# huangjh-pub/di-fusion

Hardware: AMD Instinct MI355X
Metric: frames/s integrate+decode+mesh, 640x480 synthetic stream (higher is better)
Workload: dtype f32

## Files before the change

### di_fusion_amd/_lib.py

```python
from __future__ import annotations

import ctypes
import os
from ctypes import POINTER, Structure, c_float, c_int32, c_int64, c_uint8, c_void_p
from pathlib import Path

PKG = Path(__file__).resolve().parent
LIB_PATH = Path(os.environ["DIF_LIB"]) if os.environ.get("DIF_LIB") else PKG / "libdifusion.so"

C_N_OCCUPIED, C_OVERFLOW, C_ALLOC_NEW, C_M, C_C, C_ITEMS, C_K, C_B, C_VH, C_T, C_QUERY_M, C_N_KEPT, C_CACHE_T, C_CACHE_KEPT, C_EXPORT_N, C_WORK, C_CACHE_DEAD, C_CACHE_LIVE, C_OPT_ROWS, C_OPT_VOXELS, C_HALO_L, C_HALO_R, C_HALO_TICKET, C_DEFERRED = range(24)
C_STAMP = 31
SYNC_FUSED, SYNC_FRONT_DONE, SYNC_WORDS = 0, 32, 64
FC_COUNT = 32
C_COUNT = 32
PROF_NAMES = ["encode", "decode_lattice", "decode_points", "mc_count", "mc_emit", "halo_export", "halo_merge"]
PROF_COUNT = 8
LATENT_DIM = 29

ERRORS = {-1: "DIF_EINVAL (bad argument)", -2: "DIF_ELAUNCH (HIP launch/runtime failure)", -3: "DIF_ENOSPACE (workspace too small)"}


class DifMap(Structure):
    _fields_ = [("nx", c_int32), ("ny", c_int32), ("nz", c_int32),
                ("bound_min", c_float * 3), ("voxel_size", c_float),
                ("prune_min_vox_obs", c_int32), ("ignore_count_th", c_float), ("encoder_count_th", c_float),
                ("capacity", c_int64),
                ("indexer", c_void_p), ("latent_vecs", c_void_p), ("latent_vecs_pos", c_void_p),
# ... 100 lines not shown
    "dif_query_decode": (c_int32, [POINTER(DifMap), POINTER(DifWeights), c_void_p, c_int64, c_void_p, c_void_p, c_void_p, c_void_p, c_void_p]),
    "dif_query_grad_scatter": (c_int32, [c_void_p, c_void_p, c_void_p, c_int64, c_void_p, c_void_p]),
    "dif_query_grad_gather": (c_int32, [c_void_p, c_void_p, c_void_p, c_int64, c_void_p, c_void_p]),
    "dif_export_records": (c_int32, [POINTER(DifMap), c_void_p, c_int64, c_int32, c_int32, c_int32, c_void_p, c_void_p]),
    "dif_merge_records": (c_int32, [POINTER(DifMap), c_void_p, c_int64, c_int32, c_void_p, c_void_p]),
    "dif_export_halo": (c_int32, [POINTER(DifMap), c_void_p, c_int64, c_int32, c_int32, c_void_p, c_void_p]),
    "dif_merge_halo": (c_int32, [POINTER(DifMap), c_void_p, c_int64, c_void_p, c_void_p]),
    "dif_export_halo_delta": (c_int32, [POINTER(DifMap), c_void_p, c_void_p, c_int64, c_void_p, c_void_p]),
    "dif_halo_lists_reset": (c_int32, [POINTER(DifMap), c_void_p, c_void_p, c_void_p, c_void_p]),
    "dif_merge_halo2": (c_int32, [POINTER(DifMap), c_void_p, c_int64, c_void_p, c_int64, c_void_p, c_void_p, c_void_p]),
    "dif_profile_enable": (c_int32, [c_int32]),
    "dif_profile_read": (c_int32, [POINTER(ctypes.c_double), POINTER(c_int64), c_int32]),
    "dif_profile_dump": (c_int64, [POINTER(c_int32), POINTER(c_float), c_int64, c_int32]),
    "dif_read_counters": (c_int32, [POINTER(DifMap), POINTER(c_int32), c_void_p]),
    "dif_test_mc_grid_cap": (c_int32, [c_int32]),
    "dif_test_sdma_mode": (c_int32, [c_int32]),
    "dif_sdma_info": (c_int32, [POINTER(c_int32)]),
    "dif_test_handoff": (c_int32, [c_int32, c_int32, c_int32, c_int32, POINTER(c_int64)]),
    "dif_queues_independent": (c_int32, [c_void_p, c_void_p]),
    "dif_mesh_cache_export_sdma": (c_int32, [POINTER(DifExtractBuffers), c_int64, c_int64, c_void_p, c_void_p, c_void_p]),
    "dif_sdf_hg_workspace_bytes": (c_int64, [c_int64]),
    "dif_sdf_hg": (c_int32, [POINTER(DifMap), POINTER(DifWeights), c_void_p, c_int64, POINTER(DifSdfHg), c_void_p, c_int64, c_void_p, c_void_p,
                             c_int64, c_void_p]),
    "dif_gradient_xy": (c_int32, [c_void_p, c_int32, c_int32, c_void_p, c_void_p]),
    "dif_photo_pyramid": (c_int32, [c_void_p, c_void_p, c_int32, c_int32, POINTER(DifPhotoPyramid), c_void_p]),
    "dif_rgb_odometry": (c_int32, [c_void_p, c_void_p, c_void_p, c_void_p, c_void_p, c_int32, c_int32, POINTER(DifRgbHg), c_void_p, c_void_p,
                                   c_void_p]),
    "dif_rgb_hg_workspace_bytes": (c_int64, []),
    "dif_rgb_hg": (c_int32, [c_void_p, c_void_p, c_void_p, c_void_p, c_void_p, c_int32, c_int32, POINTER(DifRgbHg), c_void_p, c_int64, c_void_p,
                             c_void_p, c_int64, c_void_p]),
# ... 67 lines not shown
```

### di_fusion_amd/csrc/difusion.hip

```cpp
#include <cstdlib>
#include <cstdio>
#include <cstring>
#include <mutex>
#include <atomic>
#include <chrono>
#include <vector>
#include <hip/hip_runtime.h>
#include <hsa/hsa.h>
#include <hsa/hsa_ext_amd.h>
#include <dlfcn.h>

#include "common.hip.h"
#include "mlp.hip.h"
#include "mc_tables.inc"

using namespace dif;

namespace {

constexpr int L = DIF_LATENT_DIM;

__device__ __constant__ int c_mc_edge_table[256];
__device__ __constant__ unsigned long long c_mc_tri_packed[256];
bool g_tables_uploaded[64] = {};
// ... 442 lines not shown
    }
    return DIF_OK;
}

static int integrate_impl(const dif_map_t* map, const dif_weights_t* w, const float* xyz, const float* normal, int64_t N, uint8_t* unq_mask,
                          void* wsp, int64_t ws_bytes, const FrameSource* src, void* stream_) {
    if (!map || !w || !w->enc_packed || w->enc_packed_floats != ENC_FLOATS || N < 0 || !map->grid_tot) return DIF_EINVAL;
    if (N == 0) return DIF_OK;
    if (!src && (!xyz || !normal)) return DIF_EINVAL;
    IntegratePlan P;
    const int rc = integrate_plan(map, w, xyz, normal, N, unq_mask, wsp, ws_bytes, src, P);
    if (rc != DIF_OK) return rc;
    hipStream_t s = (hipStream_t)stream_;
    const int nb_pts = (int)((N + DIF_BLOCK - 1) / DIF_BLOCK);
    const int nb_x = P.has_pending ? DIF_EXPORT_WGS : 0;
    if (P.overlap && wait_word(s, map->sync_words + DIF_SYNC_FUSED, map->frame_seq - 1) != DIF_OK) return DIF_ELAUNCH;
    if (src)
        hipLaunchKernelGGL(k_unproject_voxel_count, dim3(nb_pts + nb_x), dim3(DIF_BLOCK), 0, s, P.uvc, ImageGeo{src->H, src->W, src->fx, src->fy, src->cx, src->cy}, nb_x);
    else
        hipLaunchKernelGGL(k_voxel_count, dim3(nb_pts), dim3(DIF_BLOCK), 0, s, P.uvc.g, xyz, N, P.uvc.pt_lin, P.uvc.frame_count, P.uvc.counters, P.uvc.px_lo,
                           P.uvc.px_hi);
    hipLaunchKernelGGL(k_prune_mark, dim3(nb_pts + nb_x), dim3(DIF_BLOCK), 0, s, P.prune, N, nb_x);
    DIF_CHECK_LAUNCH();
    if (launch_counted_scan(P.alloc, (int)((P.grid + 31) / 32), P.alloc_tot, s) != DIF_OK) return DIF_ELAUNCH;
    hipLaunchKernelGGL(k_focus_gather, dim3(nb_pts + nb_x), dim3(DIF_BLOCK), 0, s, P.gather, N, (src && src->W % 16 == 0 && src->H % 16 == 0) ? src->W : 0, nb_x);
    DIF_CHECK_LAUNCH();
    {
        const bool x6 = w->enc_x6_packed && w->enc_x6_packed_bytes == E6_BYTES;
        const size_t lds_bytes = x6 ? (size_t)E6_BYTES : (size_t)ENC_FLOATS * 4;
        if (encoder_attributes() != DIF_OK) return DIF_ELAUNCH;
        const EncArgs& e = P.enc;
        ProfScope prof(DIF_PROF_ENCODE, s);
        const int enc_grid = P.overlap ? overlap_encoder_cus() : num_cus();
        if (x6)
            hipLaunchKernelGGL(k_encode<true>, dim3(enc_grid), dim3(ENC_X6_THREADS), lds_bytes, s, e.g, (const float*)w->enc_x6_packed, e.src.xyz, e.src.normal, e.src.frame,
                               e.src.im, N, e.pair_list, e.rec_dir, e.rec_next, e.rec, e.upd_list, e.counters, e.dirty, e.dirty_tot);
        else
            hipLaunchKernelGGL(k_encode<false>, dim3(enc_grid), dim3(512), lds_bytes, s, e.g, w->enc_packed, e.src.xyz, e.src.normal, e.src.frame,
                               e.src.im, N, e.pair_list, e.rec_dir, e.rec_next, e.rec, e.upd_list, e.counters, e.dirty, e.dirty_tot);
        DIF_CHECK_LAUNCH();
    }
    hipStream_t sf = s;
    if (P.overlap) {
        sf = (hipStream_t)map->fuse_stream;
        hipLaunchKernelGGL(k_publish_word, dim3(1), dim3(64), 0, s, map->sync_words + DIF_SYNC_FRONT_DONE, (uint32_t)map->frame_seq);
        if (wait_word(sf, map->sync_words + DIF_SYNC_FRONT_DONE, map->frame_seq) != DIF_OK) return DIF_ELAUNCH;
    }
    hipLaunchKernelGGL(k_fuse, dim3(grid_for(map->capacity * 32, DIF_BLOCK, 256)), dim3(DIF_BLOCK), 0, sf, P.fuse);
    DIF_CHECK_LAUNCH();
    return DIF_OK;
}

int dif_integrate(const dif_map_t* map, const dif_weights_t* w, const float* xyz, const float* normal, int64_t N, uint8_t* unq_mask,
                  void* wsp, int64_t ws_bytes, void* stream_) {
    return integrate_impl(map, w, xyz, normal, N, unq_mask, wsp, ws_bytes, nullptr, stream_);
}

int dif_integrate_frame(const dif_map_t* map, const dif_weights_t* w, const dif_frame_t* frame_dev, int32_t H, int32_t W, float fx, float fy, float cx,
                        float cy, float* xyz_world, float* normal_world, uint8_t* unq_mask, void* wsp, int64_t ws_bytes, void* stream_) {
    if (!frame_dev || H <= 0 || W <= 0 || (xyz_world == nullptr) != (normal_world == nullptr)) return DIF_EINVAL;
    FrameSource src{frame_dev, H, W, fx, fy, cx, cy};
    return integrate_impl(map, w, xyz_world, normal_world, (int64_t)H * W, unq_mask, wsp, ws_bytes, &src, stream_);
}
// ... 368 lines not shown
}

static void mc_onepass_args(McArgs& a, const dif_map_t* map, const dif_extract_buffers_t* buf, bool defer) {
    a.tri_start = map->tri_start; a.tri_n = map->tri_n; a.tri_count = buf->tri_count; a.tri_offset = nullptr;
    if (!defer && buf->out_tri && buf->out_id && buf->out_std) {
        a.out_tri = buf->out_tri; a.out_id = buf->out_id; a.out_std = buf->out_std; a.out_capacity = buf->out_capacity;
    }
}

static FinishArgs finish_args_of(const dif_map_t* map, const dif_extract_buffers_t* buf, bool fused_scan, bool onepass, bool exported, bool defer) {
    int32_t* const super_sum = buf->chunk_sum ? buf->chunk_sum + (buf->max_voxels + 255) / 256 : nullptr;
    const bool ov = overlapped(map);
    return FinishArgs{buf->occ_slot, map->vbm, map->counters, buf->max_triangles, buf->cache_capacity, buf->cache_tri, buf->cache_id, buf->cache_std,
                      ExtractOut{buf->counters_out, buf->out_tri, buf->out_id, buf->out_std, buf->out_capacity, (exported || defer) ? 1 : 0,
                                 defer ? (dif_pending_export_t*)map->pending_export : nullptr, buf->stamp, defer ? buf->export_notify : nullptr},
                      (fused_scan && !onepass) ? buf->chunk_sum : nullptr, super_sum, map->dirty_tot, (int)((map->capacity + DIF_BLOCK - 1) / DIF_BLOCK),
                      onepass ? buf->mc_status : nullptr, onepass ? buf->mc_status + (buf->max_voxels + 3) / 4 : nullptr,
                      ov ? map->frame_counters : nullptr};
}

static int voxel_decode_attributes() {
    static bool attr_set[64] = {};
    int dev = 0; (void)hipGetDevice(&dev);
    if (dev < 64 && !attr_set[dev]) {
        const int fp32_bytes = (int)(((size_t)((DEC_LDS_FLOATS + 3) & ~3) + 4 * VD_WAVE_LDS_FLOATS) * 4);
        const int x6_bytes = (int)((size_t)X6_LDS_BYTES + 4 * VD_WAVE_LDS_FLOATS * 4);
        if (hipFuncSetAttribute((const void*)k_decode_voxels<false>, hipFuncAttributeMaxDynamicSharedMemorySize, fp32_bytes) != hipSuccess) return DIF_ELAUNCH;
        if (hipFuncSetAttribute((const void*)k_decode_voxels<true>, hipFuncAttributeMaxDynamicSharedMemorySize, x6_bytes) != hipSuccess) return DIF_ELAUNCH;
        if (hipFuncSetAttribute((const void*)k_decode_refine_x6, hipFuncAttributeMaxDynamicSharedMemorySize, (int)X6_LDS_BYTES) != hipSuccess) return DIF_ELAUNCH;
        if (hipFuncSetAttribute((const void*)k_decode_voxels_batch<true>, hipFuncAttributeMaxDynamicSharedMemorySize, x6_bytes) != hipSuccess) return DIF_ELAUNCH;
        if (hipFuncSetAttribute((const void*)k_decode_refine_x6_batch, hipFuncAttributeMaxDynamicSharedMemorySize, (int)X6_LDS_BYTES) != hipSuccess) return DIF_ELAUNCH;
        attr_set[dev] = true;
    }
    return DIF_OK;
}

static std::atomic<int> g_mc_grid_cap{0};
int dif_test_mc_grid_cap(int32_t n) { return g_mc_grid_cap.exchange(n > 0 ? n : 0); }

static int mc_onepass_setup(const McArgs& a, size_t& lds_bytes, int& grid1, int64_t max_voxels) {
    if (upload_tables() != DIF_OK) return DIF_ELAUNCH;
    const int r = a.R / 2, nc = (r + 1) * (r + 1) * (r + 1);
    lds_bytes = (size_t)(DIF_BLOCK / 64) * MC_ONEPASS_WAVE_LDS_FLOATS(nc) * sizeof(float);
    if (lds_bytes > 128 * 1024) return DIF_EINVAL;
    static bool attr_set1[64] = {};
    int dev = 0; (void)hipGetDevice(&dev);
    if (dev < 64 && !attr_set1[dev]) {
        if (hipFuncSetAttribute((const void*)k_marching_cubes_onepass<0>, hipFuncAttributeMaxDynamicSharedMemorySize, 128 * 1024) != hipSuccess) return DIF_ELAUNCH;
        if (hipFuncSetAttribute((const void*)k_marching_cubes_onepass<4>, hipFuncAttributeMaxDynamicSharedMemorySize, 128 * 1024) != hipSuccess) return DIF_ELAUNCH;
        if (hipFuncSetAttribute((const void*)k_marching_cubes_onepass_batch<0>, hipFuncAttributeMaxDynamicSharedMemorySize, 128 * 1024) != hipSuccess) return DIF_ELAUNCH;
        if (hipFuncSetAttribute((const void*)k_marching_cubes_onepass_batch<4>, hipFuncAttributeMaxDynamicSharedMemorySize, 128 * 1024) != hipSuccess) return DIF_ELAUNCH;
        attr_set1[dev] = true;
    }
// ... 15 lines not shown
    const int* n_slots = map->counters + DIF_C_N_OCCUPIED;
    if (!map->grid_tot) return DIF_EINVAL;
    const GridMarks bits = grid_marks_of(map);
    if (buf->cache_capacity <= 0 || buf->cache_capacity >= ((int64_t)1 << 31) || !buf->cache_tri || !buf->cache_id || !buf->cache_std || !buf->cache_alive)
        return DIF_EINVAL;
    if (!map->tri_start || !map->tri_n) return DIF_EINVAL;
    hipStream_t s = (hipStream_t)stream_;
    const int64_t grid = (int64_t)map->nx * map->ny * map->nz;
    Geo g = geo_of(map);
    int* C = map->counters;
    const bool ov = overlapped(map);
    if (ov && (!overlap_ok(map) || no_cache || defer_export_of(map, buf) || s != (hipStream_t)map->fuse_stream)) return DIF_EINVAL;
    const ExtractGeo e = extract_geo(resolution);
    const int r = e.r, R = e.R, l = e.l, R3 = e.R3;
    if (buf->max_voxels * (int64_t)R3 >= ((int64_t)1 << 31)) return DIF_EINVAL;
    const double sample_a = e.sample_a, sample_b = e.sample_b;

    {
        const DirtySet ds = dirty_set_of(map, buf, no_cache);
        const bool tiled = ds.tiled;
        if (tiled) {
            hipLaunchKernelGGL(k_mark_halo_dirty, dim3(grid_for(map->capacity, DIF_BLOCK, 256)), dim3(DIF_BLOCK), 0, s, g, map->ignore_count_th, map->dirty,
                               (const int64_t*)map->latent_vecs_pos, (const int64_t*)map->indexer, (const float*)map->voxel_obs_count, bits,
                               n_slots, ds.own_lin_lo, ds.own_lin_hi);
            DIF_CHECK_LAUNCH();
        }
        {
            DirtyFunctor f{ds};
            if (map->dirty_tot && !no_cache && !tiled && map->capacity > 4096 && map->capacity % DIF_BLOCK == 0) {
                hipLaunchKernelGGL(k_dirty_scan, dim3((int)(map->capacity / DIF_BLOCK)), dim3(DIF_BLOCK), 0, s, ds, n_slots, (const int*)map->dirty_tot,
                                   ov ? map->sync_words + DIF_SYNC_FUSED : nullptr, (int)map->frame_seq);
                DIF_CHECK_LAUNCH();
            } else if (ov) {
                return DIF_EINVAL;
            } else if (map->dirty_tot && !no_cache && !tiled) {
                if (launch_counted_scan_bounded(f, n_slots, map->capacity, map->dirty_tot, s) != DIF_OK) return DIF_ELAUNCH;
            } else if (launch_scan(f, n_slots, 0, map->capacity, buf->block_tmp, s) != DIF_OK) return DIF_ELAUNCH;
        }
    }
    {
        OccFunctor f{map->grid_bits, map->indexer, buf->occ_slot, map->vbm, C, buf->max_voxels};
        if (launch_counted_scan(f, (int)((grid + 31) / 32), map->grid_tot, s) != DIF_OK) return DIF_ELAUNCH;
    }
    int rc;
    if (fast && l * l * l <= VD_MAX_L3 && R * R <= VD_MAX_R2) {
        if (!w->dec_packed || w->dec_packed_floats != DEC_FLOATS) return DIF_EINVAL;
        const bool fold = w->dec_fold_packed && w->dec_fold_packed_floats == DECF_FLOATS && buf->fold_table;
        const VoxelDecodeArgs V = voxel_decode_args_of(map, w, buf, e, fold);
        const bool x6 = fold && w->dec_x6_packed && w->dec_x6_packed_bytes == X6_BYTES;
        const size_t lds_bytes = x6 ? (size_t)X6_LDS_BYTES + 4 * VD_WAVE_LDS_FLOATS * 4
                                    : ((size_t)((DEC_LDS_FLOATS + 3) & ~3) + 4 * VD_WAVE_LDS_FLOATS) * 4;
        if (voxel_decode_attributes() != DIF_OK) return DIF_ELAUNCH;
        int64_t blocks = (buf->max_voxels + 3) / 4;
        if (blocks > num_cus()) blocks = num_cus();
        {
            ProfScope prof(DIF_PROF_DECODE_LATTICE, s);
            if (x6) hipLaunchKernelGGL(k_decode_voxels<true>, dim3((int)blocks), dim3(512), lds_bytes, s, V, (const float*)w->dec_x6_packed);
            else hipLaunchKernelGGL(k_decode_voxels<false>, dim3((int)blocks), dim3(512), lds_bytes, s, V, w->dec_packed);
        }
        DIF_CHECK_LAUNCH();
        const DecodeArgs Rf = refine_args_of(map, buf, e, fold);
        if (x6) {
            int64_t rblocks = (buf->max_voxels * (int64_t)(R3 / 32) + 7) / 8;
// ... 32 lines not shown
    return extract_mesh_part(map, buf, e, max_std, no_cache, scale_vertices, s);
}

static int extract_mesh_part(const dif_map_t* map, const dif_extract_buffers_t* buf, const ExtractGeo& e, float max_std, int32_t no_cache,
                             int32_t scale_vertices, hipStream_t s) {
    int* C = map->counters;
    const int r = e.r;
    int rc;
    McArgs a = mc_args_of(map, buf, e, max_std, scale_vertices);
    if (no_cache) {
        if (hipMemsetAsync(C + DIF_C_CACHE_T, 0, sizeof(int), s) != hipSuccess) return DIF_ELAUNCH;
        if (hipMemsetAsync(C + DIF_C_CACHE_DEAD, 0, sizeof(int), s) != hipSuccess) return DIF_ELAUNCH;
        if (hipMemsetAsync(map->tri_n, 0, sizeof(int32_t) * (size_t)map->capacity, s) != hipSuccess) return DIF_ELAUNCH;
    }
    const bool defer = defer_export_of(map, buf);
    const bool fused_scan = buf->chunk_sum && buf->max_voxels <= ((int64_t)1 << 24);
    int32_t* const super_sum = buf->chunk_sum ? buf->chunk_sum + (buf->max_voxels + 255) / 256 : nullptr;
    const bool onepass = fused_scan && buf->mc_status && r * r * r <= 64;
    if (onepass) {
        mc_onepass_args(a, map, buf, defer);
        size_t lds_bytes; int grid1;
        rc = mc_onepass_setup(a, lds_bytes, grid1, buf->max_voxels);
        if (rc != DIF_OK) return rc;
        {
            ProfScope prof(DIF_PROF_MC_COUNT, s);
            if (r == 4) hipLaunchKernelGGL(k_marching_cubes_onepass<4>, dim3(grid1), dim3(DIF_BLOCK), lds_bytes, s, a, buf->mc_status, buf->mc_status + (buf->max_voxels + 3) / 4);
            else hipLaunchKernelGGL(k_marching_cubes_onepass<0>, dim3(grid1), dim3(DIF_BLOCK), lds_bytes, s, a, buf->mc_status, buf->mc_status + (buf->max_voxels + 3) / 4);
        }
        DIF_CHECK_LAUNCH();
    } else if (fused_scan) {
        a.chunk_sum = buf->chunk_sum; a.super_sum = super_sum; a.tri_start = map->tri_start; a.tri_n = map->tri_n;
        a.tri_count = buf->tri_count; a.tri_offset = nullptr;
        size_t lds_bytes; int blocks;
        rc = mc_setup(a, lds_bytes, blocks, buf->max_voxels);
        if (rc != DIF_OK) return rc;
        {
            ProfScope prof(DIF_PROF_MC_COUNT, s);
            hipLaunchKernelGGL(k_marching_cubes<false>, dim3(blocks), dim3(DIF_BLOCK), lds_bytes, s, a);
        }
        {
            ProfScope prof(DIF_PROF_MC_EMIT, s);
            hipLaunchKernelGGL(k_marching_cubes<true>, dim3(blocks), dim3(DIF_BLOCK), lds_bytes, s, a);
        }
        DIF_CHECK_LAUNCH();
    } else {
        TriScanFunctor ts{};
        ts.valid_blocks = buf->valid_blocks; ts.indexer = map->indexer; ts.tri_start = map->tri_start; ts.tri_n = map->tri_n; ts.alive = buf->cache_alive;
        ts.new_limit = buf->max_triangles; ts.capacity = buf->cache_capacity;
        rc = mc_count_and_scan(a, buf->max_voxels, buf->tri_count, buf->tri_offset, buf->block_tmp, C, ts, s);
        if (rc != DIF_OK) return rc;
        rc = mc_emit(a, buf->max_voxels, buf->tri_count, buf->tri_offset, s);
        if (rc != DIF_OK) return rc;
    }
    hipLaunchKernelGGL(k_extract_finish, dim3(grid_for(buf->max_voxels, DIF_BLOCK, 256)), dim3(DIF_BLOCK), 0, s,
                       finish_args_of(map, buf, fused_scan, onepass, onepass && a.out_tri, defer));
    DIF_CHECK_LAUNCH();
    return DIF_OK;
}

int dif_extract_streams(const dif_stream_frame_t* st, int32_t S, const dif_weights_t* w, int32_t resolution, float max_std, int32_t scale_vertices,
                        void* stream_) {
    if (!batch_maps_ok(st, S) || !w || resolution < 1 || resolution > 4) return DIF_EINVAL;
    const ExtractGeo e = extract_geo(resolution);
    if (e.l * e.l * e.l > VD_MAX_L3 || e.R * e.R > VD_MAX_R2 || e.r * e.r * e.r > 64) return DIF_EINVAL;
    if (!w->dec_packed || w->dec_packed_floats != DEC_FLOATS || !w->dec_fold_packed || w->dec_fold_packed_floats != DECF_FLOATS || !w->dec_x6_packed ||
        w->dec_x6_packed_bytes != X6_BYTES)
        return DIF_EINVAL;
    const dif_map_t* m0 = st[0].map;
// ... 706 lines not shown
```

### di_fusion_amd/csrc/kernels_extract.hip.h

```cpp
#pragma once

__device__ __forceinline__ void mark_confident_nbhd(const Geo& g, int lin, float ignore_th, const int64_t* __restrict__ indexer,
                                                    const float* __restrict__ obs, const GridMarks& marks) {
    const uint32_t* bits = marks.bits;
    int ix, iy, iz;
    unlinearize(g, lin, ix, iy, iz);
    int cand[7];
    cand[0] = lin;
    cand[1] = linearize(g, clampi(ix - 1, 0, g.nx - 1), iy, iz);
    cand[2] = linearize(g, clampi(ix + 1, 0, g.nx - 1), iy, iz);
    cand[3] = linearize(g, ix, clampi(iy - 1, 0, g.ny - 1), iz);
    cand[4] = linearize(g, ix, clampi(iy + 1, 0, g.ny - 1), iz);
    cand[5] = linearize(g, ix, iy, clampi(iz - 1, 0, g.nz - 1));
    cand[6] = linearize(g, ix, iy, clampi(iz + 1, 0, g.nz - 1));
    int64_t slot[7];
#pragma unroll
    for (int c = 0; c < 7; ++c) slot[c] = indexer[cand[c]];
    float w[7];
#pragma unroll
    for (int c = 0; c < 7; ++c) w[c] = slot[c] >= 0 ? obs[slot[c]] : ignore_th;
    uint32_t word[7];
#pragma unroll
    for (int c = 0; c < 7; ++c) word[c] = (w[c] > ignore_th) ? bits[cand[c] >> 5] : 0xFFFFFFFFu;
    uint32_t prev[7];
// ... 47 lines not shown
    __device__ int count(int s) const { return ((a.no_cache || a.dirty[s]) && a.owned(s)) ? 1 : 0; }
    __device__ void emit(int s, int offset) const {
        a.dirty[s] = 0;
        if (offset >= a.max_voxels) return;
        const int lin = (int)a.pos[s];
        a.valid_blocks[offset] = lin;
        mark_confident_nbhd(a.g, lin, a.ignore_th, a.indexer, a.obs, a.bits);
    }
    __device__ void finish(int total) const {
        if (total > a.max_voxels) { total = (int)a.max_voxels; a.counters[DIF_C_OVERFLOW] = 2; }
        a.counters[DIF_C_K] = total;
        a.counters[DIF_C_DEFERRED] = 0;
    }
};

__device__ __forceinline__ void dirty_scan_body(const DirtySet& a, const int* __restrict__ n_ptr, const int* __restrict__ block_tot,
                                                uint32_t* __restrict__ fused_word, int seq) {
    __shared__ int smem[8];
    if (fused_word && blockIdx.x == 0 && threadIdx.x == 0) __hip_atomic_store(fused_word, (uint32_t)seq, __ATOMIC_RELAXED, __HIP_MEMORY_SCOPE_AGENT);
    const int s = (int)blockIdx.x * DIF_BLOCK + (int)threadIdx.x;
    const bool flag = a.dirty[s] != 0;
    if (!__syncthreads_or((int)flag) && blockIdx.x != 0) return;
    int before = 0, all = 0;
    const int n_blk = (int)gridDim.x;
    for (int b = (int)threadIdx.x; b < n_blk; b += DIF_BLOCK) {
        const int t = block_tot[b];
        all += t;
        if (b < (int)blockIdx.x) before += t;
    }
    const GridMarks& marks = a.bits;
    int lin = 0, cand[7];
    uint32_t word[7];
#pragma unroll
    for (int c = 0; c < 7; ++c) { cand[c] = 0; word[c] = 0xFFFFFFFFu; }
// ... 40 lines not shown
                prev[c] = (word[c] & b) ? 0xFFFFFFFFu : atomicOr(marks.bits + (cand[c] >> 5), b);
            }
#pragma unroll
            for (int c = 0; c < 7; ++c)
                if (!(prev[c] & (1u << (cand[c] & 31)))) atomicAdd(marks.tot + (cand[c] >> 5) / marks.per_words, 1);
        }
    }
    if (blockIdx.x == 0 && threadIdx.x == 0) {
        int t = total;
        if (t > a.max_voxels) { t = (int)a.max_voxels; a.counters[DIF_C_OVERFLOW] = 2; }
        a.counters[DIF_C_K] = t;
        a.counters[DIF_C_DEFERRED] = 0;
    }
}

__global__ void __launch_bounds__(DIF_BLOCK) k_dirty_scan(DirtySet a, const int* __restrict__ n_ptr, const int* __restrict__ block_tot, uint32_t* __restrict__ fused_word, int seq) {
    dirty_scan_body(a, n_ptr, block_tot, fused_word, seq);
}
struct DirtyScanArgs { DirtySet a; const int* n_ptr; const int* block_tot; };
__global__ void __launch_bounds__(DIF_BLOCK) k_dirty_scan_batch(Batch<DirtyScanArgs> b) {
    const DirtyScanArgs& a = b.s[blockIdx.y];
    dirty_scan_body(a.a, a.n_ptr, a.block_tot, nullptr, 0);
}
__global__ void k_publish_word(uint32_t* __restrict__ word, uint32_t value) {
    if (threadIdx.x == 0) __hip_atomic_store(word, value, __ATOMIC_RELAXED, __HIP_MEMORY_SCOPE_AGENT);
}

struct OccFunctor {
    uint32_t* bits;
    const int64_t* indexer;
    int32_t* occ_slot;
    int32_t* vbm;
    int* counters;
    int64_t max_voxels;
    __device__ int count(int w) const { return __popc(bits[w]); }
    __device__ void emit(int w, int offset) const {
        uint32_t word = bits[w];
// ... 374 lines not shown
        __syncthreads();
    }
}

struct VoxelDecodeArgs {
    const int32_t* occ_slot;
    const float* latent;
    Lattice low;
    int R;
    float* cube_sdf;
    float* cube_std;
    int32_t* refine_list;
    int* counters;
    const float* fold_w;
    float* fold_table;
};

#define VD_MAX_L3 64
#define VD_MAX_R2 64
#define VD_WAVE_LDS_FLOATS (2 * VD_MAX_L3 + 2 * 256)

#ifdef DIF_TRACE
__device__ unsigned long long g_vd_trace[2048 * 8];
#define VD_STAMP(slot) do { if (lane_id() == 0) g_vd_trace[((threadIdx.x >> 6) * gridDim.x + blockIdx.x) * 8 + (slot)] = wall_clock64(); } while (0)
#else
#define VD_STAMP(slot) do { } while (0)
#endif

template <bool X6, int NS>
__device__ __forceinline__ void decode_voxels_body(const BatchN<VoxelDecodeArgs, NS>& AB, int S, const float* __restrict__ wblob) {
// ... 117 lines not shown
            int32_t* const refine_list = A.refine_list;
            while (sel) {
                const int jz = __ffs((int)sel) - 1;
                sel &= sel - 1;
                refine_list[o++] = (int32_t)(e0 + jz);
            }
        }
        __syncthreads();
        VD_STAMP(4);
    }
    VD_STAMP(5);
}

template <bool X6>
__global__ void __launch_bounds__(512, X6 ? 1 : 2) k_decode_voxels(VoxelDecodeArgs A, const float* __restrict__ wblob) {
    const BatchN<VoxelDecodeArgs, 1> B{{A}};
    decode_voxels_body<X6, 1>(B, 1, wblob);
}
template <bool X6>
__global__ void __launch_bounds__(512, X6 ? 1 : 2) k_decode_voxels_batch(Batch<VoxelDecodeArgs> B, int S, const float* __restrict__ wblob) {
    decode_voxels_body<X6, DIF_MAX_STREAMS>(B, S, wblob);
}
```

### di_fusion_amd/csrc/kernels_mesh.hip.h

```cpp
#pragma once

struct McArgs {
    const int64_t* indexer; int nx, ny, nz;
    const int64_t* valid_blocks; const int* K_ptr; int64_t K_static;
    const int32_t* vbm; int64_t V;
    const float* cube_sdf; const float* cube_std; int R;
    float max_std;
    int64_t max_triangles;
    float* triangles; int64_t* tri_id; float* tri_std; uint8_t* tri_alive;
    int32_t* tri_count; const int32_t* tri_offset;
    const int* base_ptr;
    float* corner_cache; int64_t corner_stride;
    int* log_counters;
    int64_t new_limit;
    int scale; float vs, bx, by, bz;
    int32_t* chunk_sum; int32_t* super_sum; int32_t* tri_start; int32_t* tri_n;
    int* grid_tot;
    float* out_tri; int64_t* out_id; float* out_std; int64_t out_capacity;
};

__device__ __forceinline__ int mc_batch_of(const McArgs& a, int bx, int by, int bz) {
    if ((unsigned)bx >= (unsigned)a.nx || (unsigned)by >= (unsigned)a.ny || (unsigned)bz >= (unsigned)a.nz) return -1;
    int64_t vec = a.indexer[((int64_t)bx * a.ny + by) * a.nz + bz];
    if (vec == -1 || vec >= a.V) return -1;
// ... 621 lines not shown
                if (lane == 0) {
                    atomicExch(status + j, MC_ST_PREFIX | ((unsigned)(excl + aggj) & MC_ST_VALUE));
                    s_excl = excl;
                    if (j == n_groups - 1) a.log_counters[DIF_C_T] = excl + aggj;
                }
            }
            __syncthreads();
            emit_group(j, spare);
            __syncthreads();
        }
        if (exhausted && cnt == 0) break;
    }
}

template <int RC>
__device__ __forceinline__ void mc_onepass_body(const McArgs& a, unsigned* __restrict__ status, unsigned* __restrict__ ticket) {
    extern __shared__ __attribute__((aligned(16))) float lds[];
    const int K = *a.K_ptr;
    const int n_groups = (K + 3) >> 2;
    const int64_t log_n = a.log_counters[DIF_C_CACHE_T];
    if (blockIdx.x == 0) {
        if (threadIdx.x == 0) {
            a.log_counters[DIF_C_CACHE_KEPT] = (int)log_n;
            if (K == 0) a.log_counters[DIF_C_T] = 0;
        }
        if (a.grid_tot)
            for (int t = (int)threadIdx.x; t < 1024; t += (int)blockDim.x) a.grid_tot[t] = 0;
    }
    if (n_groups > (int)gridDim.x) mc_onepass_ring<RC>(a, status, ticket, lds, K, n_groups, log_n);
    else mc_onepass_direct<RC>(a, status, lds, K, n_groups, log_n);
}

template <int RC>
__global__ void __launch_bounds__(DIF_BLOCK, RC == 4 ? MC_WAVES_PER_SIMD : 4) k_marching_cubes_onepass(McArgs a, unsigned* __restrict__ status, unsigned* __restrict__ ticket) {
    mc_onepass_body<RC>(a, status, ticket);
}
struct McStream { McArgs a; unsigned* status; unsigned* ticket; };
template <int RC>
__global__ void __launch_bounds__(DIF_BLOCK, RC == 4 ? MC_WAVES_PER_SIMD : 4) k_marching_cubes_onepass_batch(Batch<McStream> b) {
    const McStream& m = b.s[blockIdx.y];
    mc_onepass_body<RC>(m.a, m.status, m.ticket);
}


__global__ void __launch_bounds__(DIF_BLOCK) k_cache_export(const float* __restrict__ tri, const int64_t* __restrict__ id, const float* __restrict__ sd,
                                                          int64_t lo, int64_t n, float* __restrict__ out_tri, int64_t* __restrict__ out_id,
                                                          float* __restrict__ out_std) {
    const int64_t stride = (int64_t)gridDim.x * blockDim.x, t0 = (int64_t)blockIdx.x * blockDim.x + threadIdx.x;
    for (int64_t j = t0; j < n * 9; j += stride) out_tri[j] = tri[lo * 9 + j];
    for (int64_t j = t0; j < n * 3; j += stride) out_std[j] = sd[lo * 3 + j];
    for (int64_t j = t0; j < n; j += stride) out_id[j] = id[lo + j];
}

struct CacheLiveFunctor {
    const float* src_tri; const int64_t* src_id; const float* src_std; const uint8_t* alive;
    float* dst_tri; int64_t* dst_id; float* dst_std;
// ... 342 lines not shown
```

### di_fusion_amd/stream.py

```python
from __future__ import annotations

import ctypes
import struct
import time
from typing import List, Optional

import numpy as np
import torch

from . import _lib
from . import synthetic as syn
from .system.map import DenseIndexedMap, _next_pow2


class FusionStream:
    HOST_OUT_TRIANGLES = 1 << 18
    SDMA_SLOW_US = 150.0
    DIRECT_SLOTS = 4

    def __init__(self, model, scene: syn.Scene, cfg: syn.MapConfig, intr: syn.Intrinsic, device: torch.device,
                 n_frames: int, deg_per_frame: float = 0.5, phase_deg: float = 0.0, orbit_radius: float = 0.3,
                 noise: bool = False, resolution: int = 4, max_n_triangles: int = int(4e6), max_std: float = 0.15,
                 initial_capacity: Optional[int] = None, tiling=None, halo_mode: str = "delta", halo_loopback: bool = False):
        self.device = device
# ... 347 lines not shown
        m = self.map
        with torch.cuda.device(self.device):
            sp = _lib.stream_ptr()
            ov = bool(self.overlap and d2h in ("dma", "none") and self.resolution <= 4 and sp.value == self._ov_main)
            if not ov:
                self._ov_leave()
            k, sl, buf, export, out = self._direct_begin(i, d2h)
            lib, w = self._d_lib, self._d_w
            H, W, fx, fy, cx, cy = self._d_args
            self.last_tensors = self._d_tens[k]
            cm = m._cmap
            if ov:
                if not self._ov_active:
                    self._ov_enter()
                self._ov_seq += 1
                cm.frame_seq, cm.fuse_stream, cm.frame_counters = self._ov_seq, sp, _lib.ptr(m._frame_counters)
            try:
                _lib.check(lib.dif_integrate_frame(ctypes.byref(cm), ctypes.byref(w), _lib.ptr(sl["frame"]), H, W, fx, fy, cx, cy, *self._pts(),
                                                   _lib.ptr(self._d_mask), _lib.ptr(m._ws), m._ws.numel(), self._fe_ptr if ov else sp), "dif_integrate_frame")
                self._direct_integrated()
                if self.tiling is not None:
                    self._exchange_halo(reserved=True)
                _lib.check(lib.dif_extract(ctypes.byref(cm), ctypes.byref(w), ctypes.byref(buf), int(self.resolution), 1, float(self.max_std), 0, 1, sp),
                           "dif_extract")
            finally:
                cm.frame_seq, cm.fuse_stream, cm.frame_counters = 0, None, None
            return self._direct_end(k, sl, buf, export, d2h, out)


class FusionStreamGroup:

    MIN_CAPACITY = 8192

    def __init__(self, streams: List[FusionStream]):
        if not 1 <= len(streams) <= _lib.MAX_STREAMS:
            raise ValueError(f"1..{_lib.MAX_STREAMS} streams per group")
        a = streams[0]
        for st in streams:
            if st.tiling is not None:
# ... 61 lines not shown
```

### di_fusion_amd/system/map.py

```python
from __future__ import annotations

import argparse
import ctypes
import functools
import logging
import threading
from pathlib import Path
from typing import Optional

import numpy as np
import torch

from .. import _lib
from ..network import utility as net_util


class MeshExtractCache:

    def __init__(self, device, owner=None):
        self.device = device
        self._owner = owner
        self._host = None

    def _fetch(self):
# ... 134 lines not shown
        self._query_ws = None
        self._halo_list = None
        self._halo_lists_stale = True

        self._grid = int(np.prod(self.n_xyz))
        if self._grid >= 2 ** 31:
            raise RuntimeError("grid too large for 32-bit linear ids")
        with torch.cuda.device(device):
            self._indexer = torch.full((self._grid,), -1, device=device, dtype=torch.long)
            self._frame_count = torch.zeros((self._grid,), device=device, dtype=torch.int32)
            self._grid_bits = torch.zeros(((self._grid + 31) // 32,), device=device, dtype=torch.int32)
            self._grid_tot = torch.zeros((1024,), device=device, dtype=torch.int32)
            self._alloc_bits = torch.zeros(((self._grid + 31) // 32,), device=device, dtype=torch.int32)
            self._alloc_tot = torch.zeros((1024,), device=device, dtype=torch.int32)
            self._sync_words = torch.zeros((_lib.SYNC_WORDS,), device=device, dtype=torch.int32)
            self._frame_counters = torch.zeros((_lib.FC_COUNT,), device=device, dtype=torch.int32)
            self._counters = torch.zeros((_lib.C_COUNT,), device=device, dtype=torch.int32)
            self._pending_export = torch.zeros((32,), device=device, dtype=torch.int32)
        self._capacity = 0
        self._alloc_state(_next_pow2(max(int(initial_capacity), 1024)))
        self._n_occ_ub = 0
        self._ws = None
        self._ws_n = 0
        self._xbuf = None
        self._host_counters = (ctypes.c_int32 * _lib.C_COUNT)()
        self._pinned_counters = None
        self._pending_seq = 0
        self._add_total = 0
        self.last_counters = {}

    def _alloc_state(self, capacity: int):
# ... 635 lines not shown
```

### include/difusion.h

```cpp
#ifndef DIFUSION_H
#define DIFUSION_H

#include <stdint.h>

#ifdef __cplusplus
extern "C" {
#endif

#define DIF_VERSION 100
#define DIF_LATENT_DIM 29

#define DIF_MAX_STREAMS 8

#define DIF_OK 0
#define DIF_EINVAL (-1)
#define DIF_ELAUNCH (-2)
#define DIF_ENOSPACE (-3)

enum {
    DIF_C_N_OCCUPIED = 0,
    DIF_C_OVERFLOW = 1,
    DIF_C_ALLOC_NEW = 2,
    DIF_C_M = 3,
    DIF_C_C = 4,
// ... 44 lines not shown
    int32_t* tri_start;
    int32_t* tri_n;
    int32_t own_x_lo, own_x_hi, halo;
    int32_t* dirty_tot;
    int32_t* halo_list;
    int32_t halo_list_cap;
    void* pending_export;
    uint32_t* alloc_bits;
    int32_t* alloc_tot;
    uint32_t* sync_words;
    int32_t frame_seq;
    void* fuse_stream;
    int32_t* frame_counters;
} dif_map_t;

enum { DIF_SYNC_FUSED = 0, DIF_SYNC_FRONT_DONE = 32, DIF_SYNC_WORDS = 64 };
enum { DIF_FC_SHADOW = 4, DIF_FC_COUNT = 32 };

typedef struct dif_pending_export {
    int32_t pending, kept, n, seq;
    const float* log_tri; const int64_t* log_id; const float* log_std;
    float* out_tri; int64_t* out_id; float* out_std;
    int32_t* notify;
} dif_pending_export_t;

typedef struct dif_weights {
    const float* enc_packed;
    int64_t enc_packed_floats;
    const float* dec_packed;
    int64_t dec_packed_floats;
    const float* dec_bwd_packed;
// ... 183 lines not shown

enum { DIF_PROF_ENCODE = 0, DIF_PROF_DECODE_LATTICE = 1, DIF_PROF_DECODE_POINTS = 2, DIF_PROF_MC_COUNT = 3, DIF_PROF_MC_EMIT = 4,
       DIF_PROF_HALO_EXPORT = 5 , DIF_PROF_HALO_MERGE = 6 ,
       DIF_PROF_COUNT = 8 };
int dif_profile_enable(int32_t on);
int dif_profile_read(double* ms , int64_t* launches , int32_t reset);
int64_t dif_profile_dump(int32_t* which , float* ms , int64_t capacity, int32_t reset);

int dif_read_counters(const dif_map_t* map, int32_t* host_out , void* stream);

int dif_queues_independent(void* stream_a, void* stream_b);

int dif_mesh_cache_export_sdma(const dif_extract_buffers_t* buf, int64_t lo, int64_t n, float* out_tri, int64_t* out_id, float* out_std);

int dif_test_mc_grid_cap(int32_t n);
int dif_test_sdma_mode(int32_t mode);
int dif_test_handoff(int32_t mode, int32_t groups, int32_t iters, int32_t flags, int64_t* out);
int dif_sdma_info(int32_t* out);

#ifdef __cplusplus
}
#endif
#endif
```

Measured before the change: 9982.

## Restructure overlapped frame pipeline: fuse waits on decode completion, extract waits on fuse

Moves the cross-frame synchronisation point so that the front half of integration for frame N runs without waiting on the previous frame. Only k_fuse now waits on a DECODED word, which marching cubes publishes once decode has finished reading latents. Fuse runs on the main stream and publishes FUSE_DONE, and extract waits on that word. frame_counters is double-buffered by frame parity, and dirty_tot clearing moves into the decode kernel so the dirty scan no longer publishes. A test delay hook and an exception cleanup path are also added. The risk is subtle ordering hazards between fuse and the previous frame's extract.

```diff
diff --git a/di_fusion_amd/_lib.py b/di_fusion_amd/_lib.py
--- a/di_fusion_amd/_lib.py
+++ b/di_fusion_amd/_lib.py
@@ -10,7 +10,7 @@
 
 C_N_OCCUPIED, C_OVERFLOW, C_ALLOC_NEW, C_M, C_C, C_ITEMS, C_K, C_B, C_VH, C_T, C_QUERY_M, C_N_KEPT, C_CACHE_T, C_CACHE_KEPT, C_EXPORT_N, C_WORK, C_CACHE_DEAD, C_CACHE_LIVE, C_OPT_ROWS, C_OPT_VOXELS, C_HALO_L, C_HALO_R, C_HALO_TICKET, C_DEFERRED = range(24)
 C_STAMP = 31
-SYNC_FUSED, SYNC_FRONT_DONE, SYNC_WORDS = 0, 32, 64
+SYNC_DECODED, SYNC_FUSE_DONE, SYNC_WORDS = 0, 32, 64
 FC_COUNT = 32
 C_COUNT = 32
 PROF_NAMES = ["encode", "decode_lattice", "decode_points", "mc_count", "mc_emit", "halo_export", "halo_merge"]
@@ -141,6 +141,7 @@
     "dif_profile_dump": (c_int64, [POINTER(c_int32), POINTER(c_float), c_int64, c_int32]),
     "dif_read_counters": (c_int32, [POINTER(DifMap), POINTER(c_int32), c_void_p]),
     "dif_test_mc_grid_cap": (c_int32, [c_int32]),
+    "dif_test_extract_delay": (c_int32, [c_int32]),
     "dif_test_sdma_mode": (c_int32, [c_int32]),
     "dif_sdma_info": (c_int32, [POINTER(c_int32)]),
     "dif_test_handoff": (c_int32, [c_int32, c_int32, c_int32, c_int32, POINTER(c_int64)]),
diff --git a/di_fusion_amd/csrc/difusion.hip b/di_fusion_amd/csrc/difusion.hip
--- a/di_fusion_amd/csrc/difusion.hip
+++ b/di_fusion_amd/csrc/difusion.hip
@@ -480,7 +480,6 @@
     hipStream_t s = (hipStream_t)stream_;
     const int nb_pts = (int)((N + DIF_BLOCK - 1) / DIF_BLOCK);
     const int nb_x = P.has_pending ? DIF_EXPORT_WGS : 0;
-    if (P.overlap && wait_word(s, map->sync_words + DIF_SYNC_FUSED, map->frame_seq - 1) != DIF_OK) return DIF_ELAUNCH;
     if (src)
         hipLaunchKernelGGL(k_unproject_voxel_count, dim3(nb_pts + nb_x), dim3(DIF_BLOCK), 0, s, P.uvc, ImageGeo{src->H, src->W, src->fx, src->fy, src->cx, src->cy}, nb_x);
     else
@@ -506,13 +505,9 @@
                                e.src.im, N, e.pair_list, e.rec_dir, e.rec_next, e.rec, e.upd_list, e.counters, e.dirty, e.dirty_tot);
         DIF_CHECK_LAUNCH();
     }
-    hipStream_t sf = s;
-    if (P.overlap) {
-        sf = (hipStream_t)map->fuse_stream;
-        hipLaunchKernelGGL(k_publish_word, dim3(1), dim3(64), 0, s, map->sync_words + DIF_SYNC_FRONT_DONE, (uint32_t)map->frame_seq);
-        if (wait_word(sf, map->sync_words + DIF_SYNC_FRONT_DONE, map->frame_seq) != DIF_OK) return DIF_ELAUNCH;
-    }
-    hipLaunchKernelGGL(k_fuse, dim3(grid_for(map->capacity * 32, DIF_BLOCK, 256)), dim3(DIF_BLOCK), 0, sf, P.fuse);
+    if (P.overlap && wait_word(s, map->sync_words + DIF_SYNC_DECODED, map->frame_seq - 1) != DIF_OK) return DIF_ELAUNCH;
+    hipLaunchKernelGGL(k_fuse, dim3(grid_for(map->capacity * 32, DIF_BLOCK, 256)), dim3(DIF_BLOCK), 0, s, P.fuse);
+    if (P.overlap) hipLaunchKernelGGL(k_publish_word, dim3(1), dim3(64), 0, s, map->sync_words + DIF_SYNC_FUSE_DONE, (uint32_t)map->frame_seq);
     DIF_CHECK_LAUNCH();
     return DIF_OK;
 }
@@ -911,7 +906,7 @@
     return FinishArgs{buf->occ_slot, map->vbm, map->counters, buf->max_triangles, buf->cache_capacity, buf->cache_tri, buf->cache_id, buf->cache_std,
                       ExtractOut{buf->counters_out, buf->out_tri, buf->out_id, buf->out_std, buf->out_capacity, (exported || defer) ? 1 : 0,
                                  defer ? (dif_pending_export_t*)map->pending_export : nullptr, buf->stamp, defer ? buf->export_notify : nullptr},
-                      (fused_scan && !onepass) ? buf->chunk_sum : nullptr, super_sum, map->dirty_tot, (int)((map->capacity + DIF_BLOCK - 1) / DIF_BLOCK),
+                      (fused_scan && !onepass) ? buf->chunk_sum : nullptr, super_sum, ov ? nullptr : map->dirty_tot, (int)((map->capacity + DIF_BLOCK - 1) / DIF_BLOCK),
                       onepass ? buf->mc_status : nullptr, onepass ? buf->mc_status + (buf->max_voxels + 3) / 4 : nullptr,
                       ov ? map->frame_counters : nullptr};
 }
@@ -934,6 +929,11 @@
 
 static std::atomic<int> g_mc_grid_cap{0};
 int dif_test_mc_grid_cap(int32_t n) { return g_mc_grid_cap.exchange(n > 0 ? n : 0); }
+static std::atomic<int> g_extract_delay_us{0};
+int dif_test_extract_delay(int32_t us) { return g_extract_delay_us.exchange(us <= 0 ? 0 : us > 500 ? 500 : us); }
+
+static bool mc_fused_scan(const dif_extract_buffers_t* buf) { return buf->chunk_sum && buf->max_voxels <= ((int64_t)1 << 24); }
+static bool mc_takes_onepass(const dif_extract_buffers_t* buf, int r) { return mc_fused_scan(buf) && buf->mc_status && r * r * r <= 64; }
 
 static int mc_onepass_setup(const McArgs& a, size_t& lds_bytes, int& grid1, int64_t max_voxels) {
     if (upload_tables() != DIF_OK) return DIF_ELAUNCH;
@@ -979,6 +979,8 @@
     const ExtractGeo e = extract_geo(resolution);
     const int r = e.r, R = e.R, l = e.l, R3 = e.R3;
     if (buf->max_voxels * (int64_t)R3 >= ((int64_t)1 << 31)) return DIF_EINVAL;
+    if (ov && !(fast && l * l * l <= VD_MAX_L3 && R * R <= VD_MAX_R2 && mc_takes_onepass(buf, r))) return DIF_EINVAL;
+    if (ov && wait_word(s, map->sync_words + DIF_SYNC_FUSE_DONE, map->frame_seq) != DIF_OK) return DIF_ELAUNCH;
     const double sample_a = e.sample_a, sample_b = e.sample_b;
 
     {
@@ -993,8 +995,8 @@
         {
             DirtyFunctor f{ds};
             if (map->dirty_tot && !no_cache && !tiled && map->capacity > 4096 && map->capacity % DIF_BLOCK == 0) {
-                hipLaunchKernelGGL(k_dirty_scan, dim3((int)(map->capacity / DIF_BLOCK)), dim3(DIF_BLOCK), 0, s, ds, n_slots, (const int*)map->dirty_tot,
-                                   ov ? map->sync_words + DIF_SYNC_FUSED : nullptr, (int)map->frame_seq);
+                hipLaunchKernelGGL(k_dirty_scan, dim3((int)(map->capacity / DIF_BLOCK)), dim3(DIF_BLOCK), 0, s, ds,
+                                   ov ? (const int*)map->frame_counters + DIF_FC_SHADOW : n_slots, (const int*)map->dirty_tot);
                 DIF_CHECK_LAUNCH();
             } else if (ov) {
                 return DIF_EINVAL;
@@ -1011,7 +1013,10 @@
     if (fast && l * l * l <= VD_MAX_L3 && R * R <= VD_MAX_R2) {
         if (!w->dec_packed || w->dec_packed_floats != DEC_FLOATS) return DIF_EINVAL;
         const bool fold = w->dec_fold_packed && w->dec_fold_packed_floats == DECF_FLOATS && buf->fold_table;
-        const VoxelDecodeArgs V = voxel_decode_args_of(map, w, buf, e, fold);
+        VoxelDecodeArgs V = voxel_decode_args_of(map, w, buf, e, fold);
+        if (ov) {
+            V.dirty_tot = map->dirty_tot; V.n_dirty_tot = (int)((map->capacity + DIF_BLOCK - 1) / DIF_BLOCK);
+        }
         const bool x6 = fold && w->dec_x6_packed && w->dec_x6_packed_bytes == X6_BYTES;
         const size_t lds_bytes = x6 ? (size_t)X6_LDS_BYTES + 4 * VD_WAVE_LDS_FLOATS * 4
                                     : ((size_t)((DEC_LDS_FLOATS + 3) & ~3) + 4 * VD_WAVE_LDS_FLOATS) * 4;
@@ -1074,18 +1079,22 @@
         if (hipMemsetAsync(map->tri_n, 0, sizeof(int32_t) * (size_t)map->capacity, s) != hipSuccess) return DIF_ELAUNCH;
     }
     const bool defer = defer_export_of(map, buf);
-    const bool fused_scan = buf->chunk_sum && buf->max_voxels <= ((int64_t)1 << 24);
+    const bool fused_scan = mc_fused_scan(buf);
     int32_t* const super_sum = buf->chunk_sum ? buf->chunk_sum + (buf->max_voxels + 255) / 256 : nullptr;
-    const bool onepass = fused_scan && buf->mc_status && r * r * r <= 64;
+    const bool onepass = mc_takes_onepass(buf, r);
+    if (overlapped(map) && !onepass) return DIF_EINVAL;
     if (onepass) {
         mc_onepass_args(a, map, buf, defer);
+        uint32_t* const decoded_word = overlapped(map) ? map->sync_words + DIF_SYNC_DECODED : nullptr;
         size_t lds_bytes; int grid1;
         rc = mc_onepass_setup(a, lds_bytes, grid1, buf->max_voxels);
         if (rc != DIF_OK) return rc;
         {
             ProfScope prof(DIF_PROF_MC_COUNT, s);
-            if (r == 4) hipLaunchKernelGGL(k_marching_cubes_onepass<4>, dim3(grid1), dim3(DIF_BLOCK), lds_bytes, s, a, buf->mc_status, buf->mc_status + (buf->max_voxels + 3) / 4);
-            else hipLaunchKernelGGL(k_marching_cubes_onepass<0>, dim3(grid1), dim3(DIF_BLOCK), lds_bytes, s, a, buf->mc_status, buf->mc_status + (buf->max_voxels + 3) / 4);
+            if (r == 4) hipLaunchKernelGGL(k_marching_cubes_onepass<4>, dim3(grid1), dim3(DIF_BLOCK), lds_bytes, s, decoded_word, (uint32_t)map->frame_seq, a, buf->mc_status,
+                                           buf->mc_status + (buf->max_voxels + 3) / 4);
+            else hipLaunchKernelGGL(k_marching_cubes_onepass<0>, dim3(grid1), dim3(DIF_BLOCK), lds_bytes, s, decoded_word, (uint32_t)map->frame_seq, a, buf->mc_status,
+                                    buf->mc_status + (buf->max_voxels + 3) / 4);
         }
         DIF_CHECK_LAUNCH();
     } else if (fused_scan) {
@@ -1112,6 +1121,8 @@
         rc = mc_emit(a, buf->max_voxels, buf->tri_count, buf->tri_offset, s);
         if (rc != DIF_OK) return rc;
     }
+    if (const int us = g_extract_delay_us.load(std::memory_order_relaxed))
+        hipLaunchKernelGGL(k_test_spin, dim3(1), dim3(64), 0, s, (unsigned long long)us * 100ull);
     hipLaunchKernelGGL(k_extract_finish, dim3(grid_for(buf->max_voxels, DIF_BLOCK, 256)), dim3(DIF_BLOCK), 0, s,
                        finish_args_of(map, buf, fused_scan, onepass, onepass && a.out_tri, defer));
     DIF_CHECK_LAUNCH();
diff --git a/di_fusion_amd/csrc/kernels_extract.hip.h b/di_fusion_amd/csrc/kernels_extract.hip.h
--- a/di_fusion_amd/csrc/kernels_extract.hip.h
+++ b/di_fusion_amd/csrc/kernels_extract.hip.h
@@ -85,10 +85,8 @@
     }
 };
 
-__device__ __forceinline__ void dirty_scan_body(const DirtySet& a, const int* __restrict__ n_ptr, const int* __restrict__ block_tot,
-                                                uint32_t* __restrict__ fused_word, int seq) {
+__device__ __forceinline__ void dirty_scan_body(const DirtySet& a, const int* __restrict__ n_ptr, const int* __restrict__ block_tot) {
     __shared__ int smem[8];
-    if (fused_word && blockIdx.x == 0 && threadIdx.x == 0) __hip_atomic_store(fused_word, (uint32_t)seq, __ATOMIC_RELAXED, __HIP_MEMORY_SCOPE_AGENT);
     const int s = (int)blockIdx.x * DIF_BLOCK + (int)threadIdx.x;
     const bool flag = a.dirty[s] != 0;
     if (!__syncthreads_or((int)flag) && blockIdx.x != 0) return;
@@ -159,13 +157,18 @@
     }
 }
 
-__global__ void __launch_bounds__(DIF_BLOCK) k_dirty_scan(DirtySet a, const int* __restrict__ n_ptr, const int* __restrict__ block_tot, uint32_t* __restrict__ fused_word, int seq) {
-    dirty_scan_body(a, n_ptr, block_tot, fused_word, seq);
+__global__ void __launch_bounds__(DIF_BLOCK) k_dirty_scan(DirtySet a, const int* __restrict__ n_ptr, const int* __restrict__ block_tot) {
+    dirty_scan_body(a, n_ptr, block_tot);
 }
 struct DirtyScanArgs { DirtySet a; const int* n_ptr; const int* block_tot; };
 __global__ void __launch_bounds__(DIF_BLOCK) k_dirty_scan_batch(Batch<DirtyScanArgs> b) {
     const DirtyScanArgs& a = b.s[blockIdx.y];
-    dirty_scan_body(a.a, a.n_ptr, a.block_tot, nullptr, 0);
+    dirty_scan_body(a.a, a.n_ptr, a.block_tot);
+}
+__global__ void k_test_spin(unsigned long long ticks) {
+    if (threadIdx.x != 0) return;
+    const unsigned long long t0 = wall_clock64();
+    while (wall_clock64() - t0 < ticks) __builtin_amdgcn_s_sleep(16);
 }
 __global__ void k_publish_word(uint32_t* __restrict__ word, uint32_t value) {
     if (threadIdx.x == 0) __hip_atomic_store(word, value, __ATOMIC_RELAXED, __HIP_MEMORY_SCOPE_AGENT);
@@ -570,6 +573,7 @@
     int* counters;
     const float* fold_w;
     float* fold_table;
+    int32_t* dirty_tot; int n_dirty_tot;
 };
 
 #define VD_MAX_L3 64
@@ -717,6 +721,8 @@
 
 template <bool X6>
 __global__ void __launch_bounds__(512, X6 ? 1 : 2) k_decode_voxels(VoxelDecodeArgs A, const float* __restrict__ wblob) {
+    if (A.dirty_tot && A.counters[DIF_C_DEFERRED] == 0)
+        for (int t = (int)(blockIdx.x * blockDim.x + threadIdx.x); t < A.n_dirty_tot; t += (int)(gridDim.x * blockDim.x)) A.dirty_tot[t] = 0;
     const BatchN<VoxelDecodeArgs, 1> B{{A}};
     decode_voxels_body<X6, 1>(B, 1, wblob);
 }
diff --git a/di_fusion_amd/csrc/kernels_mesh.hip.h b/di_fusion_amd/csrc/kernels_mesh.hip.h
--- a/di_fusion_amd/csrc/kernels_mesh.hip.h
+++ b/di_fusion_amd/csrc/kernels_mesh.hip.h
@@ -659,13 +659,15 @@
 }
 
 template <int RC>
-__device__ __forceinline__ void mc_onepass_body(const McArgs& a, unsigned* __restrict__ status, unsigned* __restrict__ ticket) {
+__device__ __forceinline__ void mc_onepass_body(const McArgs& a, unsigned* __restrict__ status, unsigned* __restrict__ ticket,
+                                                uint32_t* __restrict__ decoded_word, uint32_t seq) {
     extern __shared__ __attribute__((aligned(16))) float lds[];
     const int K = *a.K_ptr;
     const int n_groups = (K + 3) >> 2;
     const int64_t log_n = a.log_counters[DIF_C_CACHE_T];
     if (blockIdx.x == 0) {
         if (threadIdx.x == 0) {
+            if (decoded_word) __hip_atomic_store(decoded_word, seq, __ATOMIC_RELAXED, __HIP_MEMORY_SCOPE_AGENT);
             a.log_counters[DIF_C_CACHE_KEPT] = (int)log_n;
             if (K == 0) a.log_counters[DIF_C_T] = 0;
         }
@@ -677,14 +679,15 @@
 }
 
 template <int RC>
-__global__ void __launch_bounds__(DIF_BLOCK, RC == 4 ? MC_WAVES_PER_SIMD : 4) k_marching_cubes_onepass(McArgs a, unsigned* __restrict__ status, unsigned* __restrict__ ticket) {
-    mc_onepass_body<RC>(a, status, ticket);
+__global__ void __launch_bounds__(DIF_BLOCK, RC == 4 ? MC_WAVES_PER_SIMD : 4) k_marching_cubes_onepass(uint32_t* __restrict__ decoded_word, uint32_t seq, McArgs a, unsigned* __restrict__ status,
+                                                                                                   unsigned* __restrict__ ticket) {
+    mc_onepass_body<RC>(a, status, ticket, decoded_word, seq);
 }
 struct McStream { McArgs a; unsigned* status; unsigned* ticket; };
 template <int RC>
 __global__ void __launch_bounds__(DIF_BLOCK, RC == 4 ? MC_WAVES_PER_SIMD : 4) k_marching_cubes_onepass_batch(Batch<McStream> b) {
     const McStream& m = b.s[blockIdx.y];
-    mc_onepass_body<RC>(m.a, m.status, m.ticket);
+    mc_onepass_body<RC>(m.a, m.status, m.ticket, nullptr, 0u);
 }
 
 
diff --git a/di_fusion_amd/stream.py b/di_fusion_amd/stream.py
--- a/di_fusion_amd/stream.py
+++ b/di_fusion_amd/stream.py
@@ -385,7 +385,7 @@
                 if not self._ov_active:
                     self._ov_enter()
                 self._ov_seq += 1
-                cm.frame_seq, cm.fuse_stream, cm.frame_counters = self._ov_seq, sp, _lib.ptr(m._frame_counters)
+                cm.frame_seq, cm.fuse_stream, cm.frame_counters = self._ov_seq, sp, ctypes.c_void_p(m._frame_counters.data_ptr() + 4 * _lib.FC_COUNT * (self._ov_seq & 1))
             try:
                 _lib.check(lib.dif_integrate_frame(ctypes.byref(cm), ctypes.byref(w), _lib.ptr(sl["frame"]), H, W, fx, fy, cx, cy, *self._pts(),
                                                    _lib.ptr(self._d_mask), _lib.ptr(m._ws), m._ws.numel(), self._fe_ptr if ov else sp), "dif_integrate_frame")
@@ -394,6 +394,9 @@
                     self._exchange_halo(reserved=True)
                 _lib.check(lib.dif_extract(ctypes.byref(cm), ctypes.byref(w), ctypes.byref(buf), int(self.resolution), 1, float(self.max_std), 0, 1, sp),
                            "dif_extract")
+            except Exception:
+                self._ov_leave()
+                raise
             finally:
                 cm.frame_seq, cm.fuse_stream, cm.frame_counters = 0, None, None
             return self._direct_end(k, sl, buf, export, d2h, out)
diff --git a/di_fusion_amd/system/map.py b/di_fusion_amd/system/map.py
--- a/di_fusion_amd/system/map.py
+++ b/di_fusion_amd/system/map.py
@@ -172,7 +172,7 @@
             self._alloc_bits = torch.zeros(((self._grid + 31) // 32,), device=device, dtype=torch.int32)
             self._alloc_tot = torch.zeros((1024,), device=device, dtype=torch.int32)
             self._sync_words = torch.zeros((_lib.SYNC_WORDS,), device=device, dtype=torch.int32)
-            self._frame_counters = torch.zeros((_lib.FC_COUNT,), device=device, dtype=torch.int32)
+            self._frame_counters = torch.zeros((2, _lib.FC_COUNT), device=device, dtype=torch.int32)
             self._counters = torch.zeros((_lib.C_COUNT,), device=device, dtype=torch.int32)
             self._pending_export = torch.zeros((32,), device=device, dtype=torch.int32)
         self._capacity = 0
diff --git a/include/difusion.h b/include/difusion.h
--- a/include/difusion.h
+++ b/include/difusion.h
@@ -82,7 +82,7 @@
     int32_t* frame_counters;
 } dif_map_t;
 
-enum { DIF_SYNC_FUSED = 0, DIF_SYNC_FRONT_DONE = 32, DIF_SYNC_WORDS = 64 };
+enum { DIF_SYNC_DECODED = 0, DIF_SYNC_FUSE_DONE = 32, DIF_SYNC_WORDS = 64 };
 enum { DIF_FC_SHADOW = 4, DIF_FC_COUNT = 32 };
 
 typedef struct dif_pending_export {
@@ -296,6 +296,7 @@
 int dif_mesh_cache_export_sdma(const dif_extract_buffers_t* buf, int64_t lo, int64_t n, float* out_tri, int64_t* out_id, float* out_std);
 
 int dif_test_mc_grid_cap(int32_t n);
+int dif_test_extract_delay(int32_t us);
 int dif_test_sdma_mode(int32_t mode);
 int dif_test_handoff(int32_t mode, int32_t groups, int32_t iters, int32_t flags, int64_t* out);
 int dif_sdma_info(int32_t* out);
```

Measured after the change: 9015. 0.903x the previous value.
